# linum-uqam/ViT-OCM-WMSegmentation

Hardware: AMD Instinct MI355X
Metric: OCM tiles/s (224x224, ViT-S/16 attention-map inference) (higher is better)
Workload: dtype bf16x3

## Files before the change

### include/ocm_vit.h

```cpp
#ifndef OCM_VIT_H
#define OCM_VIT_H

#include <stddef.h>
#include <stdint.h>

#ifdef __cplusplus
extern "C" {
#endif

#define OCM_ABI_VERSION 20

enum {
    OCM_OK = 0,
    OCM_EINVAL = 1,
    OCM_ESTATE = 2,
    OCM_EHIP = 3,
    OCM_ENOMEM = 4,
    OCM_ENAME = 5
};

enum {
    OCM_PREC_BF16 = 0,
    OCM_PREC_FP32 = 1,
    OCM_PREC_BF16X3 = 2
// ... 101 lines not shown
int ocm_linear_resid_ln_supported(int32_t D);
int ocm_op_linear_resid_ln(int32_t precision, const void *a, const void *w, const float *bias, const float *resid,
                           float *x, const float *gamma, const float *beta, void *xn, int32_t M, int32_t D, int32_t K,
                           float eps, void *stream);

enum { OCM_GEMM_LINEAR = 0, OCM_GEMM_QKV = 1, OCM_GEMM_LINEAR_LD = 2, OCM_GEMM_CONV = 3, OCM_GEMM_RESID_LN = 4 };
enum { OCM_PLAN_STATS_EPILOGUE = 1, OCM_PLAN_SPLITK_OFFERED = 2, OCM_PLAN_CONV3X3 = 4 };
typedef struct ocm_gemm_plan_info {
    int32_t bm, bn;
    int32_t waves;
    int32_t mfma16;
    int32_t lds_dma;
    int32_t stages;
    int32_t ksteps;
    int32_t splitk;
} ocm_gemm_plan_info;
int ocm_gemm_plan(int32_t family, int32_t precision, int32_t epilogue, int32_t M, int32_t N, int32_t K, uint32_t flags,
                  ocm_gemm_plan_info *plan);

int32_t ocm_n_pad(int32_t n_tokens);
int32_t ocm_n_pad_prec(int32_t precision, int32_t n_tokens);

int ocm_op_qkv_proj(int32_t precision, const void *a, const void *w, const float *bias, void *q, void *k,
                    void *vt, float *qkv_f32, int32_t batch, int32_t n_tokens, int32_t heads,
                    void *stream);

int ocm_op_attention(int32_t precision, const void *q, const void *k, const void *vt, void *ctx, float *lse2,
                     int32_t batch, int32_t n_tokens, int32_t heads, float scale, void *stream);

int ocm_op_attention_probs(int32_t precision, const void *q, const void *k, const float *lse2, float *attn,
                           int32_t batch, int32_t n_tokens, int32_t heads, float scale,
                           void *stream);

int ocm_op_attention_rows(int32_t precision, const void *q, const void *k, const int32_t *query_rows,
                          int32_t n_rows, float *rows, int32_t batch, int32_t n_tokens, int32_t heads, float scale,
                          void *stream);

int ocm_op_qkv_proj_hd(int32_t precision, const void *a, const void *w, const float *bias, void *q, void *k, void *vt,
                       float *qkv_f32, int32_t batch, int32_t n_tokens, int32_t heads, int32_t head_dim, void *stream);
int ocm_op_attention_hd(int32_t precision, const void *q, const void *k, const void *vt, void *ctx, float *lse2,
                        int32_t batch, int32_t n_tokens, int32_t heads, int32_t head_dim, float scale, void *stream);
int ocm_op_attention_probs_hd(int32_t precision, const void *q, const void *k, const float *lse2, float *attn,
                              int32_t batch, int32_t n_tokens, int32_t heads, int32_t head_dim, float scale, void *stream);

enum {
    OCM_ATTN_BF16_WHOLE = 0,
    OCM_ATTN_BF16_STREAM = 1,
    OCM_ATTN_FP32_STREAM = 2,
    OCM_ATTN_X3_WAVE_SPLIT = 3,
    OCM_ATTN_X3_PIPELINED = 4,
    OCM_ATTN_X3_DMA = 5,
    OCM_ATTN_X3_DMA_KSPLIT = 6
};
typedef struct ocm_attention_plan_info {
    int32_t kernel;
    int32_t waves;
    int32_t stages;
    int32_t kslices;
    int32_t grid_x, grid_y, grid_z;
    int32_t lds_bytes;
    uint64_t workspace_need;
} ocm_attention_plan_info;
int ocm_attention_plan(int32_t precision, int32_t batch, int32_t n_tokens, int32_t heads, int32_t head_dim, size_t workspace_bytes,
                       ocm_attention_plan_info *plan);

size_t ocm_attention_workspace_bytes(int32_t precision, int32_t batch, int32_t n_tokens, int32_t heads, int32_t head_dim);
// ... 231 lines not shown
```

### vit-ocm-wmsegmentation_amd/_lib.py

```python
import ctypes as C
import os

_HERE = os.path.dirname(os.path.abspath(__file__))
LIB_PATH = os.environ.get("OCM_VIT_LIB") or os.path.join(_HERE, "libocm_vit.so")

OCM_ABI_VERSION = 20
OCM_OK, OCM_EINVAL, OCM_ESTATE, OCM_EHIP, OCM_ENOMEM, OCM_ENAME = 0, 1, 2, 3, 4, 5

OCM_PREC_BF16 = 0
OCM_PREC_FP32 = 1
OCM_PREC_BF16X3 = 2
OCM_SWIN_OPT_FUSE_MLP = 0
OCM_SWIN_CFG_BACKBONE = 1
OCM_SWIN_OUT_HIDDEN, OCM_SWIN_OUT_RESHAPED, OCM_SWIN_OUT_ATTENTION = 0, 1, 2
PRECISIONS = {"bf16": OCM_PREC_BF16, "fp32": OCM_PREC_FP32, "bf16x3": OCM_PREC_BF16X3}
DEFAULT_PRECISION = "bf16x3"
OCM_LN_F32, OCM_LN_BF16, OCM_LN_SPLIT = 0, 1, 2
OCM_OPT_FUSE_LN = 0
OCM_OPT_FOLD_LN = 1

OCM_OUT_FEAT = 1 << 0
OCM_OUT_ATTN = 1 << 1
OCM_OUT_QKV = 1 << 2
OCM_OUT_TOKENS = 1 << 3
# ... 109 lines not shown
    "ocm_abi_version": (C.c_int, []),
    "ocm_last_error": (C.c_char_p, []),
    "ocm_vit_create": (C.c_int, [C.POINTER(OcmVitConfig), C.POINTER(_vp)]),
    "ocm_vit_destroy": (None, [_vp]),
    "ocm_vit_set_param": (C.c_int, [_vp, C.c_char_p, _vp, _sz, _vp]),
    "ocm_vit_params_ready": (C.c_int, [_vp]),
    "ocm_vit_workspace_bytes": (_sz, [_vp, _i32, _i32]),
    "ocm_vit_forward": (C.c_int, [_vp, C.POINTER(OcmVitIO)]),
    "ocm_vit_prepare_tokens": (C.c_int, [_vp, C.POINTER(OcmVitIO), _vp]),
    "ocm_vit_block_forward": (C.c_int, [_vp, _i32, _vp, _i32, _i32, _i32, _vp, _vp, _vp, _sz, _vp]),
    "ocm_vit_final_norm": (C.c_int, [_vp, _vp, _vp, _i64, _vp]),
    "ocm_op_layernorm": (C.c_int, [_vp, _vp, _vp, _vp, _i32, _i64, _i32, _f32, _vp]),
    "ocm_op_cast_bf16": (C.c_int, [_vp, _vp, _sz, _vp]),
    "ocm_op_cast_split": (C.c_int, [_vp, _vp, _sz, _vp]),
    "ocm_op_merge_split": (C.c_int, [_vp, _vp, _sz, _vp]),
    "ocm_n_pad_prec": (_i32, [_i32, _i32]),
    "ocm_op_linear": (C.c_int, [_i32, _vp, _vp, _vp, _vp, _vp, _i32, _i32, _i32, _i32, _vp]),
    "ocm_op_linear_stats": (C.c_int, [_i32, _vp, _vp, _vp, _vp, _vp, _vp, _vp, _vp, _vp, _i32, _i32, _i32, _vp]),
    "ocm_linear_resid_ln_supported": (C.c_int, [_i32]),
    "ocm_op_linear_resid_ln": (C.c_int, [_i32, _vp, _vp, _vp, _vp, _vp, _vp, _vp, _vp, _i32, _i32, _i32, _f32, _vp]),
    "ocm_gemm_plan": (C.c_int, [_i32, _i32, _i32, _i32, _i32, _i32, C.c_uint32, C.POINTER(OcmGemmPlanInfo)]),
    "ocm_n_pad": (_i32, [_i32]),
    "ocm_op_qkv_proj": (C.c_int, [_i32, _vp, _vp, _vp, _vp, _vp, _vp, _vp, _i32, _i32, _i32, _vp]),
    "ocm_op_attention": (C.c_int, [_i32, _vp, _vp, _vp, _vp, _vp, _i32, _i32, _i32, _f32, _vp]),
    "ocm_op_qkv_proj_hd": (C.c_int, [_i32, _vp, _vp, _vp, _vp, _vp, _vp, _vp, _i32, _i32, _i32, _i32, _vp]),
    "ocm_op_attention_hd": (C.c_int, [_i32, _vp, _vp, _vp, _vp, _vp, _i32, _i32, _i32, _i32, _f32, _vp]),
    "ocm_op_attention_probs_hd": (C.c_int, [_i32, _vp, _vp, _vp, _vp, _i32, _i32, _i32, _i32, _f32, _vp]),
    "ocm_attention_plan": (C.c_int, [_i32, _i32, _i32, _i32, _i32, _sz, C.POINTER(OcmAttentionPlanInfo)]),
    "ocm_attention_workspace_bytes": (_sz, [_i32, _i32, _i32, _i32, _i32]),
    "ocm_op_attention_ws": (C.c_int, [_i32, _vp, _vp, _vp, _vp, _vp, _i32, _i32, _i32, _i32, _f32, _vp, _sz, _vp]),
    "ocm_op_attention_generic": (C.c_int, [C.c_int32, C.c_void_p, C.c_void_p, C.c_void_p, C.c_int32, C.c_int32, C.c_int32,
                                           C.c_int32, C.c_float, C.c_void_p]),
    "ocm_op_attention_probs": (C.c_int, [_i32, _vp, _vp, _vp, _vp, _i32, _i32, _i32, _f32, _vp]),
    "ocm_op_attention_rows": (C.c_int, [_i32, _vp, _vp, _vp, _i32, _vp, _i32, _i32, _i32, _f32, _vp]),
    "ocm_op_attention_map": (C.c_int, [_vp, _vp, _i32, _i32, _i32, _i32, _i32, _i32, _i32, _vp]),
    "ocm_op_tile_postprocess": (C.c_int, [_vp, _vp, _i32, _i32, _i32, _i32, _vp]),
    "ocm_op_bilinear_upsample": (C.c_int, [_vp, _vp, _i32, _i32, _i32, _i32, _vp]),
    "ocm_op_nearest_upsample": (C.c_int, [_vp, _vp, _i32, _i32, _i32, _i32, _vp]),
    "ocm_op_stitch": (C.c_int, [_vp, _vp, _vp, _i32, _i32, _i32, _vp]),
    "ocm_op_normalize_u8": (C.c_int, [_vp, _i64, _vp, _vp, _vp, _vp]),
    "ocm_otsu_threshold": (_i32, [C.POINTER(C.c_uint64), _i64]),
    "ocm_op_threshold_u8": (C.c_int, [_vp, _vp, _i64, _i32, _vp]),
    "ocm_vit_graph_stats": (C.c_int, [C.c_void_p, C.POINTER(C.c_uint64), C.POINTER(C.c_uint64)]),
    "ocm_swin_create": (C.c_int, [C.POINTER(OcmSwinConfig), C.POINTER(C.c_void_p)]),
    "ocm_swin_destroy": (None, [C.c_void_p]),
    "ocm_swin_set_param": (C.c_int, [C.c_void_p, C.c_char_p, C.c_void_p, C.c_size_t, C.c_void_p]),
    "ocm_swin_params_ready": (C.c_int, [C.c_void_p]),
    "ocm_swin_workspace_bytes": (C.c_size_t, [C.c_void_p, C.c_int32]),
    "ocm_swin_forward": (C.c_int, [C.c_void_p, C.c_void_p, C.c_int32, C.c_void_p, C.c_void_p, C.c_void_p, C.c_void_p,
                                   C.c_size_t, C.c_void_p]),
    "ocm_swin_forward_ex": (C.c_int, [C.c_void_p, C.c_void_p, C.c_int32, C.c_void_p, C.c_void_p, C.c_void_p,
                                      C.POINTER(OcmSwinOutputs), C.c_void_p, C.c_size_t, C.c_void_p]),
    "ocm_swin_output_shape": (C.c_int, [C.POINTER(OcmSwinConfig), C.c_int32, C.c_int32, C.c_int32, C.POINTER(C.c_int64)]),
    "ocm_swin_set_option": (C.c_int, [C.c_void_p, C.c_int32, C.c_int32]),
    "ocm_op_swin_window_probs": (C.c_int, [C.c_int32, C.c_void_p, C.c_int32, C.c_void_p, C.c_void_p, C.c_void_p, C.c_int32,
                                           C.c_int32, C.c_int32, C.c_int32, C.c_int32, C.c_int32, C.c_void_p]),
    "ocm_swin_window_scratch_floats": (C.c_size_t, [C.c_int32, C.c_int32]),
    "ocm_op_swin_tokens_to_nchw": (C.c_int, [C.c_void_p, C.c_void_p, C.c_int32, C.c_int32, C.c_int32, C.c_void_p]),
    "ocm_op_swin_lnqkv": (C.c_int, [C.c_int32, C.c_void_p, C.c_void_p, C.c_void_p, C.c_void_p, C.c_void_p, C.c_void_p,
                                    C.c_int64, C.c_int32, C.c_float, C.c_void_p]),
    "ocm_op_swin_mlp": (C.c_int, [C.c_int32, C.c_void_p, C.c_void_p, C.c_void_p, C.c_void_p, C.c_void_p, C.c_void_p,
                                  C.c_void_p, C.c_int64, C.c_int32, C.c_int32, C.c_float, C.c_void_p]),
    "ocm_op_swin_attn_block": (C.c_int, [C.c_int32, C.c_void_p, C.c_void_p, C.c_void_p, C.c_void_p, C.c_void_p, C.c_void_p,
                                         C.c_void_p, C.c_void_p, C.c_void_p, C.c_int32, C.c_int32, C.c_int32, C.c_int32,
                                         C.c_int32, C.c_int32, C.c_float, C.c_void_p]),
    "ocm_op_swin_window_attention": (C.c_int, [C.c_int32, C.c_void_p, C.c_int32, C.c_void_p, C.c_int32, C.c_void_p,
# ... 143 lines not shown
```

### vit-ocm-wmsegmentation_amd/csrc/attn_plan.h

```cpp
#pragma once
#include <cstddef>

enum AttnKernel : int {
    ATTN_BF16_WHOLE = 0,
    ATTN_BF16_STREAM = 1,
    ATTN_F32_STREAM = 2,
    ATTN_X3_WS = 3,
    ATTN_X3_PP = 4,
    ATTN_X3_DMA = 5,
    ATTN_X3_DMA_KSPLIT = 6,
};

struct AttnPlan {
    AttnKernel kernel;
    int waves;
    int stages;
    int kslices;
    unsigned grid_x, grid_y, grid_z;
    int lds_bytes;
    size_t workspace_need;
};

constexpr int ATTN_QTILE = 32;
constexpr int ATTN_BF16_WHOLE_MAX_N = 256;
constexpr int ATTN_X3_WIDE_MIN_N = 1024;
constexpr int ATTN_X3_WS_MAX_WGS = 128;
constexpr int ATTN_KSPLIT_MAX = 4, ATTN_KSPLIT_WGS_4 = 64, ATTN_KSPLIT_WGS_3 = 96, ATTN_KSPLIT_WGS_2 = 128;
constexpr int ATTN_KSPLIT_ROW_FLOATS = 64 + 4;
constexpr int ATTN_WS_LDS = 4 * 2 * 2 * 8192;
constexpr int ATTN_F32_LDS_PER_CHANNEL = 4 * 256;

constexpr int attn_qtiles(int n_tokens) { return (n_tokens + ATTN_QTILE - 1) / ATTN_QTILE; }
constexpr long attn_wide_wgs(int batch, int n_tokens, int heads) { return (long)((attn_qtiles(n_tokens) + 7) / 8) * batch * heads; }
constexpr size_t attn_ksplit_slice_bytes(int batch, int n_tokens, int heads) {
    return (size_t)batch * heads * n_tokens * ATTN_KSPLIT_ROW_FLOATS * sizeof(float);
}

constexpr size_t attn_plan_workspace_bytes(int prec, int batch, int n_tokens, int heads, int head_dim) {
    if (prec != 2 || head_dim != 64 || n_tokens <= ATTN_X3_WIDE_MIN_N) return 0;
    if (attn_wide_wgs(batch, n_tokens, heads) > ATTN_KSPLIT_WGS_2) return 0;
    return ATTN_KSPLIT_MAX * attn_ksplit_slice_bytes(batch, n_tokens, heads);
}

inline AttnPlan attn_plan(int prec, int batch, int n_tokens, int heads, int head_dim, size_t workspace_bytes) {
    const int qtiles = attn_qtiles(n_tokens);
    const unsigned bh = (unsigned)(batch * heads), gx4 = (unsigned)((qtiles + 3) / 4);
    if (prec == 0) {
        if (head_dim == 64 && n_tokens <= ATTN_BF16_WHOLE_MAX_N) return AttnPlan{ATTN_BF16_WHOLE, 8, 1, 1, bh, 1, 1, 0, 0};
        return AttnPlan{ATTN_BF16_STREAM, 4, 2, 1, gx4, bh, 1, 0, 0};
    }
    if (prec == 1) return AttnPlan{ATTN_F32_STREAM, 4, 2, 1, gx4, bh, 1, ATTN_F32_LDS_PER_CHANNEL * head_dim, 0};
    if (head_dim == 128) return AttnPlan{ATTN_X3_DMA, 4, 2, 1, gx4, bh, 1, 0, 0};
    if (n_tokens > ATTN_X3_WIDE_MIN_N) {
        const unsigned gx8 = (unsigned)((qtiles + 7) / 8);
        if (workspace_bytes) {
            const long wgs = (long)gx8 * bh;
            const int want = wgs <= ATTN_KSPLIT_WGS_4 ? 4 : wgs <= ATTN_KSPLIT_WGS_3 ? 3 : wgs <= ATTN_KSPLIT_WGS_2 ? 2 : 1;
            const int per = (qtiles + want - 1) / want, nslice = (qtiles + per - 1) / per;
            const size_t need = (size_t)nslice * attn_ksplit_slice_bytes(batch, n_tokens, heads);
            if (nslice > 1 && need <= workspace_bytes) return AttnPlan{ATTN_X3_DMA_KSPLIT, 8, 3, nslice, gx8, bh, (unsigned)nslice, 0, need};
        }
        return AttnPlan{ATTN_X3_DMA, 8, 3, 1, gx8, bh, 1, 0, 0};
    }
// ... 4 lines not shown
```

### vit-ocm-wmsegmentation_amd/csrc/engine.hip

```cpp
#include <stdarg.h>
#include <stdio.h>
#include <string.h>

#include <atomic>
#include <mutex>
#include <string>
#include <vector>

#include "host_common.h"
#include "launch.h"
#include "attn_plan.h"
#include "otsu.h"

static thread_local std::string g_err;

int ocm_fail(int code, const char *fmt, ...) {
    char buf[512];
    va_list ap;
    va_start(ap, fmt);
    vsnprintf(buf, sizeof buf, fmt, ap);
    va_end(ap);
    g_err = buf;
    return code;
}
// ... 322 lines not shown
    w.bytes = off;
    return w;
}

extern "C" size_t ocm_vit_workspace_bytes(const ocm_vit_t *h, int32_t batch, int32_t n_tokens) {
    if (!h || batch <= 0 || n_tokens <= 1) return 0;
    return carve(h, batch, n_tokens, nullptr).bytes;
}

static int check_ws(const ocm_vit *h, int batch, int n, void *ws, size_t ws_bytes) {
    if (!ws) return fail(OCM_ENOMEM, "workspace is null");
    if ((uintptr_t)ws & 255) return fail(OCM_EINVAL, "workspace must be 256-byte aligned");
    const size_t need = carve(h, batch, n, nullptr).bytes;
    if (ws_bytes < need) return fail(OCM_ENOMEM, "workspace too small: %zu < %zu bytes", ws_bytes, need);
    return OCM_OK;
}

static int run_attention(const ocm_vit *h, const Workspace &w, int batch, int n, bool attn_only, float *out_attn, float *out_qkv,
                         const int32_t *query_rows, int n_rows, float *out_rows, const char *qkv_w, const float *qkv_b,
                         const LnFold &ln, hipStream_t s) {
    const int H = h->H, np = ocm_n_pad_for(h->prec, n), pc = h->prec;
    const float scale = h->cfg.qk_scale;
    const bool want_v = !(attn_only && !out_qkv);
    if (!h->mfma_heads()) {
        float *qkv = out_qkv ? out_qkv : w.qkv32;
        { PROF(OCM_K_QKV, s); HIP_TRY(launch_qkv(pc, w.xn, qkv_w, qkv_b, nullptr, nullptr, nullptr, qkv, batch, n, np, H, h->hd, want_v, s, ln)); }
        { PROF(OCM_K_ATTN, s); HIP_TRY(launch_attention_generic(pc, qkv, attn_only ? nullptr : w.ctx, out_attn, query_rows, n_rows, out_rows, batch, n, H, h->hd, scale, s)); }
        return OCM_OK;
    }
    void *vt_dst = want_v ? w.vt : nullptr;
    { PROF(OCM_K_QKV, s); HIP_TRY(launch_qkv(pc, w.xn, qkv_w, qkv_b, w.q, w.k, vt_dst, out_qkv, batch, n, np, H, h->hd, want_v, s, ln)); }
    if (out_rows && !out_attn) { PROF(OCM_K_PROBS, s); HIP_TRY(launch_attention_rows(pc, w.q, w.k, query_rows, n_rows, out_rows, batch, n, np, H, scale, s, h->hd)); }
    if (attn_only && !out_attn) return OCM_OK;
    { PROF(OCM_K_ATTN, s); HIP_TRY(launch_attention(pc, w.q, w.k, w.vt, attn_only ? nullptr : w.ctx, out_attn ? w.lse : nullptr, batch, n, np, H, scale, s, h->hd, w.kpart, w.kpart_bytes)); }
    if (out_attn) {
        PROF(OCM_K_PROBS, s);
        HIP_TRY(launch_attention_probs(pc, w.q, w.k, w.lse, out_attn, batch, n, np, H, scale, s, h->hd, query_rows, n_rows, out_rows));
    }
    return OCM_OK;
}

static int run_block(const ocm_vit *h, int i, const Workspace &w, float *x, int batch, int n, bool attn_only,
                     float *out_attn, float *out_qkv, const int32_t *query_rows, int n_rows, float *out_rows,
                     hipStream_t s, bool xn_ready = false, const float *next_g = nullptr, const float *next_b = nullptr,
                     bool *xn_out = nullptr) {
    const BlockP &bp = h->blk[i];
    const int D = h->D, T = batch * n;
    const float eps = h->cfg.ln_eps;
    const int pc = h->prec, lnk = ln_kind_of_prec(pc);
    const long t128 = (long)((T + 127) / 128) * (D / 128);
    const int fuse_opt = h->opt[OCM_OPT_FUSE_LN];
    const bool fuse_ln = linear_resid_ln_supported(D) && fuse_opt != 1 && ((T >= 8192 && t128 < 512) || fuse_opt == 2);
    if (xn_out) *xn_out = false;
    if (!xn_ready) { PROF(OCM_K_LN, s); HIP_TRY(launch_layernorm(x, h->ptr<float>(bp.ln1_g), h->ptr<float>(bp.ln1_b), w.xn, lnk, T, D, eps, s)); }
    if (int rc = run_attention(h, w, batch, n, attn_only, out_attn, out_qkv, query_rows, n_rows, out_rows, h->ptr<char>(bp.qkv_w),
                               h->ptr<float>(bp.qkv_b), LnFold(), s))
        return rc;
    if (attn_only) return OCM_OK;
    if (fuse_ln) {
        PROF(OCM_K_PROJ, s);
        HIP_TRY(launch_linear_resid_ln(pc, w.ctx, h->ptr<char>(bp.proj_w), h->ptr<float>(bp.proj_b), x, x, h->ptr<float>(bp.ln2_g), h->ptr<float>(bp.ln2_b), w.xn, T, D, D, eps, s));
    } else {
        { PROF(OCM_K_PROJ, s); HIP_TRY(launch_linear(pc, w.ctx, h->ptr<char>(bp.proj_w), h->ptr<float>(bp.proj_b), x, x, T, D, D, OCM_EPI_BIAS_RESID_F32, s)); }
        { PROF(OCM_K_LN, s); HIP_TRY(launch_layernorm(x, h->ptr<float>(bp.ln2_g), h->ptr<float>(bp.ln2_b), w.xn, lnk, T, D, eps, s)); }
    }
    { PROF(OCM_K_FC1, s); HIP_TRY(launch_linear(pc, w.xn, h->ptr<char>(bp.fc1_w), h->ptr<float>(bp.fc1_b), nullptr, w.hid, T, h->M, D, OCM_EPI_BIAS_GELU_BF16, s)); }
    if (fuse_ln && next_g && next_b) {
        PROF(OCM_K_FC2, s);
        HIP_TRY(launch_linear_resid_ln(pc, w.hid, h->ptr<char>(bp.fc2_w), h->ptr<float>(bp.fc2_b), x, x, next_g, next_b, w.xn, T, D, h->M, eps, s));
        if (xn_out) *xn_out = true;
// ... 407 lines not shown

extern "C" int ocm_op_attention_ws(int32_t precision, const void *q, const void *k, const void *vt, void *ctx, float *lse2,
                                   int32_t batch, int32_t n_tokens, int32_t heads, int32_t head_dim, float scale,
                                   void *workspace, size_t workspace_bytes, void *stream) {
    return op_attention(precision, q, k, vt, ctx, lse2, batch, n_tokens, heads, head_dim, scale, stream, workspace, workspace_bytes);
}

extern "C" int ocm_op_attention_generic(int32_t precision, const float *qkv_f32, void *ctx, float *attn, int32_t batch,
                                        int32_t n_tokens, int32_t heads, int32_t head_dim, float scale, void *stream) {
    int pc = 0, rc = prec_of(precision, &pc);
    if (rc) return rc;
    if (!qkv_f32 || (!ctx && !attn)) return fail(OCM_EINVAL, "null argument");
    if (batch <= 0 || n_tokens <= 0 || heads <= 0 || head_dim <= 0) return fail(OCM_EINVAL, "bad shape");
    if (head_dim % 4 || head_dim > 512 || n_tokens > 8192 || (pc == 2 && (heads * head_dim) % 32))
        return fail(OCM_EINVAL, "generic attention: head_dim %d must be a multiple of 4 up to 512, at most 8192 tokens, and "
                                "heads * head_dim a multiple of 32 for a split-bf16 context", head_dim);
    if ((int64_t)batch * heads > 65535) return fail(OCM_EINVAL, "batch * heads = %lld > 65535", (long long)batch * heads);
    HIP_TRY(launch_attention_generic(pc, qkv_f32, ctx, attn, nullptr, 0, nullptr, batch, n_tokens, heads, head_dim, scale,
                                     (hipStream_t)stream));
    return OCM_OK;
}

extern "C" int ocm_op_attention_probs(int32_t precision, const void *q, const void *k, const float *lse2, float *attn,
                                      int32_t batch, int32_t n_tokens, int32_t heads, float scale, void *stream) {
    return op_attention_probs(precision, q, k, lse2, attn, batch, n_tokens, heads, 64, scale, stream);
}

extern "C" int ocm_op_attention_probs_hd(int32_t precision, const void *q, const void *k, const float *lse2, float *attn,
                                         int32_t batch, int32_t n_tokens, int32_t heads, int32_t head_dim, float scale,
                                         void *stream) {
    return op_attention_probs(precision, q, k, lse2, attn, batch, n_tokens, heads, head_dim, scale, stream);
}

extern "C" int ocm_op_attention_rows(int32_t precision, const void *q, const void *k, const int32_t *query_rows,
                                     int32_t n_rows, float *rows, int32_t batch, int32_t n_tokens, int32_t heads,
                                     float scale, void *stream) {
    int pc = 0, rc = prec_of(precision, &pc);
    if (rc) return rc;
    if (!q || !k || !rows) return fail(OCM_EINVAL, "null argument");
    if (batch <= 0 || n_tokens <= 1 || heads <= 0 || n_rows <= 0) return fail(OCM_EINVAL, "bad shape");
    HIP_TRY(launch_attention_rows(pc, q, k, query_rows, n_rows, rows, batch, n_tokens, ocm_n_pad_for(pc, n_tokens), heads, scale,
                                  (hipStream_t)stream));
    return OCM_OK;
}

extern "C" int ocm_op_attention_map(const float *attn, float *maps, int32_t b, int32_t heads, int32_t n_tokens,
                                    int32_t query, int32_t hf, int32_t wf, int32_t p, void *stream) {
    if (!attn || !maps) return fail(OCM_EINVAL, "null argument");
    if (hf * wf + 1 != n_tokens) return fail(OCM_EINVAL, "hf*wf+1 = %d != n_tokens %d", hf * wf + 1, n_tokens);
    if (query < 0 || query >= n_tokens) return fail(OCM_EINVAL, "query %d out of range", query);
    HIP_TRY(launch_attention_map(attn, maps, b, heads, n_tokens, query, hf, wf, p, (hipStream_t)stream));
    return OCM_OK;
}

extern "C" int ocm_op_tile_postprocess(const float *rows, float *maps, int32_t tiles, int32_t heads, int32_t n_rows,
                                       int32_t pixels, void *stream) {
    if (!rows || !maps) return fail(OCM_EINVAL, "null argument");
    if (tiles <= 0 || heads <= 0 || n_rows <= 0 || pixels <= 0) return fail(OCM_EINVAL, "bad shape");
    HIP_TRY(launch_tile_postprocess(rows, maps, tiles, heads, n_rows, pixels, (hipStream_t)stream));
    return OCM_OK;
}

extern "C" int ocm_op_bilinear_upsample(const float *src, float *dst, int32_t tiles, int32_t h, int32_t w,
                                        int32_t scale, void *stream) {
    if (!src || !dst) return fail(OCM_EINVAL, "null argument");
    if (tiles <= 0 || h <= 0 || w <= 0 || scale <= 0) return fail(OCM_EINVAL, "bad shape");
// ... 162 lines not shown
```

### vit-ocm-wmsegmentation_amd/csrc/kernels_attn.hip

```cpp
#include <stdlib.h>

#include "launch.h"

#define LOG2E 1.4426950408889634f
#include "attn_plan.h"
#define OCM_VMCNT_ATTN(n) asm volatile("s_waitcnt vmcnt(%0)" ::"n"(n) : "memory")

#ifndef OCM_DEFER_MAX
#define OCM_DEFER_MAX 8.0f
#endif
__device__ __forceinline__ float defer_max_update(float &m, float cand) {
    if (__any(cand > m + OCM_DEFER_MAX)) {
        const float mn = fmaxf(m, cand);
        const float alpha = fast_exp2(m - mn);
        m = mn;
        return alpha;
    }
    return 1.0f;
}

template <bool WANT_O, int HD = 64>
__global__ __launch_bounds__(256, HD == 64 ? 3 : 2) void attn_fwd_kernel(const bf16 *__restrict__ Q, const bf16 *__restrict__ Kk,
                                                       const bf16 *__restrict__ Vt, bf16 *__restrict__ ctx,
                                                       float *__restrict__ lse2, int N, int npad, int H,
// ... 1196 lines not shown
#pragma unroll
    for (int e = 0; e < 16; ++e) lr[e] = lse2[(int64_t)bh * N + min(q0 + acc_row32(e, h), N - 1)];
    float *out = attn + (int64_t)bh * N * N;
    const int nkt = (N + 31) >> 5, per = (nkt + (int)gridDim.z - 1) / (int)gridDim.z;
    const int kt0 = (int)blockIdx.z * per, ktiles = min(nkt, kt0 + per);
    if (kt0 >= ktiles) return;
    bf16x8 kh[NQ], kl[NQ], nh[NQ], nl[NQ];
    loadrow(Kb, min(kt0 * 32 + r, N - 1), kh, kl);
    for (int kt = kt0; kt < ktiles; ++kt) {
        if (kt + 1 < ktiles) loadrow(Kb, min((kt + 1) * 32 + r, N - 1), nh, nl);
        f32x16 S;
#pragma unroll
        for (int e = 0; e < 16; ++e) S[e] = 0.f;
#pragma unroll
        for (int s = 0; s < NQ; ++s) S = mfma32x3(qh[s], ql[s], kh[s], kl[s], S);
        const int key = kt * 32 + r;
        if (key < N) {
#pragma unroll
            for (int e = 0; e < 16; ++e) {
                const int qrow = q0 + acc_row32(e, h);
                if (qrow < N) out[(int64_t)qrow * N + key] = fast_exp2(S[e] * scale2 - lr[e]);
            }
        }
#pragma unroll
        for (int s = 0; s < NQ; ++s) {
            kh[s] = nh[s];
            kl[s] = nl[s];
        }
    }
}

constexpr int PROBS_FOLD_ROWS = 8;

__global__ __launch_bounds__(256) void attn_probs_x3_span_kernel(const char *__restrict__ Q, const char *__restrict__ Kk,
                                                                 const float *__restrict__ lse2, float *__restrict__ attn,
                                                                 int N, int npad, float scale2,
                                                                 const int32_t *__restrict__ query_rows, int n_rows,
                                                                 float *__restrict__ rows) {
    constexpr int HD = 64, NQ = HD / 16, ROWB = HD * 4, PITCH = ROWB + 16, REGION = 32 * PITCH, TILEB = 32 * ROWB;
    __shared__ __attribute__((aligned(16))) char smem[4 * REGION];
    const int tid = threadIdx.x, lane = tid & 63, wave = tid >> 6;
    const int r = lane & 31, h = lane >> 5;
    int qblk, bh;
    xcd_remap2(qblk, bh);
    const int q0 = qblk * 32, nq = min(32, N - q0);
    const int nkt = (N + 31) >> 5;
    const char *Qb = Q + ((int64_t)bh * npad + q0) * ROWB;
    const char *Kb = Kk + (int64_t)bh * npad * ROWB;
    f32x4 qraw[2], kraw[2][8];
#pragma unroll
    for (int i = 0; i < 2; ++i) qraw[i] = *(const f32x4 *)(Qb + (i * 256 + tid) * 16);
#pragma unroll
    for (int t = 0; t < 2; ++t)
        if (wave + 4 * t < nkt) {
#pragma unroll
            for (int i = 0; i < 8; ++i) kraw[t][i] = *(const f32x4 *)(Kb + (int64_t)(wave + 4 * t) * TILEB + (i * 64 + lane) * 16);
        }
    float lr[16];
#pragma unroll
    for (int e = 0; e < 16; ++e) lr[e] = lse2[(int64_t)bh * N + min(q0 + acc_row32(e, h), N - 1)];
    auto stage = [&](char *region, int piece, const f32x4 &v) {
        *(f32x4 *)(region + (piece >> 4) * PITCH + (piece & 15) * 16) = v;
    };
    auto fragments = [&](const char *region, bf16x8(&hi)[NQ], bf16x8(&lo)[NQ]) {
        const char *rp = region + r * PITCH;
#pragma unroll
        for (int s = 0; s < NQ; ++s) {
            const char *p = rp + (s >> 1) * 128 + ((s & 1) * 16 + 8 * h) * 2;
            hi[s] = *(const bf16x8 *)p;
            lo[s] = *(const bf16x8 *)(p + 64);
        }
    };
    bf16x8 qh[NQ], ql[NQ];
#pragma unroll
    for (int i = 0; i < 2; ++i) stage(smem, i * 256 + tid, qraw[i]);
    lds_barrier();
    fragments(smem, qh, ql);
    lds_barrier();
    char *mine = smem + wave * REGION;
    float pr[2][16];
#pragma unroll
    for (int t = 0; t < 2; ++t) {
        const bool have = wave + 4 * t < nkt;
        if (have) {
#pragma unroll
            for (int i = 0; i < 8; ++i) stage(mine, i * 64 + lane, kraw[t][i]);
        }
        lds_barrier();
        if (have) {
            bf16x8 kh[NQ], kl[NQ];
            fragments(mine, kh, kl);
            f32x16 S;
#pragma unroll
            for (int e = 0; e < 16; ++e) S[e] = 0.f;
#pragma unroll
            for (int s = 0; s < NQ; ++s) S = mfma32x3(qh[s], ql[s], kh[s], kl[s], S);
#pragma unroll
            for (int e = 0; e < 16; ++e) pr[t][e] = fast_exp2(S[e] * scale2 - lr[e]);
        }
        lds_barrier();
    }
    float *span = attn + ((int64_t)bh * N + q0) * N;
    const int shift = (int)(((uintptr_t)span >> 2) & 3);
    float *img = (float *)smem + shift;
#pragma unroll
    for (int t = 0; t < 2; ++t) {
        const int key = (wave + 4 * t) * 32 + r;
        if (key < N) {
#pragma unroll
            for (int e = 0; e < 16; ++e) {
                const int row = acc_row32(e, h);
                if (row < nq) img[row * N + key] = pr[t][e];
            }
        }
    }
    lds_barrier();
    const int len = nq * N;
    const int lead = min((4 - shift) & 3, len), nvec = (len - lead) >> 2, tail = lead + 4 * nvec;
    if (tid < lead) span[tid] = img[tid];
    for (int i = tid; i < nvec; i += 256) *(f32x4 *)(span + lead + 4 * i) = *(const f32x4 *)(img + lead + 4 * i);
    if (tid < len - tail) span[tail + tid] = img[tail + tid];
    if (rows) {
        for (int i = 0; i < n_rows; ++i) {
            const int query = query_rows ? query_rows[i] : 0;
            if (query < q0 || query >= q0 + nq) continue;
            float *dst = rows + ((int64_t)bh * n_rows + i) * (N - 1);
            const float *src = img + (query - q0) * N + 1;
            for (int j = tid; j < N - 1; j += 256) dst[j] = src[j];
        }
    }
}


__device__ __forceinline__ void store_ctx1(int prec, char *rowp, int col, float v) {
    if (prec == 0) {
        *(bf16 *)(rowp + col * 2) = (bf16)v;
    } else if (prec == 1) {
        *(float *)(rowp + col * 4) = v;
    } else {
        bf16 hi, lo;
        split1(v, hi, lo);
        *(bf16 *)(rowp + sp_off(col)) = hi;
        *(bf16 *)(rowp + sp_off(col) + 64) = lo;
    }
}
// ... 159 lines not shown
            attn_merge_x3_kernel<64><<<dim3((unsigned)((rows + 15) / 16)), dim3(256), 0, s>>>(
                ksplit_ws, p.kslices, (char *)ctx, lse2, batch * heads, n_tokens, heads);
            break;
        }
    }
    return hipGetLastError();
}

template <int HD>
static hipError_t launch_probs_hd(int prec, const void *q, const void *k, const float *lse2, float *attn, int n_tokens, int n_pad,
                                  float scale2, dim3 grid, dim3 gridz, hipStream_t s) {
    const dim3 block(256);
    if (prec == 2)
        attn_probs_x3_kernel<HD><<<gridz, block, 0, s>>>((const char *)q, (const char *)k, lse2, attn, n_tokens, n_pad, scale2);
    else if (prec)
        attn_probs_f32_kernel<HD><<<grid, block, 0, s>>>((const float *)q, (const float *)k, lse2, attn, n_tokens, n_pad, scale2);
    else
        attn_probs_kernel<HD><<<grid, block, 0, s>>>((const bf16 *)q, (const bf16 *)k, lse2, attn, n_tokens, n_pad, scale2);
    return hipGetLastError();
}

hipError_t launch_attention_probs(int prec, const void *q, const void *k, const float *lse2, float *attn, int batch,
                                  int n_tokens, int n_pad, int heads, float scale, hipStream_t s, int head_dim,
                                  const int32_t *query_rows, int n_rows, float *rows) {
    if (head_dim != 64 && head_dim != 128) return hipErrorInvalidValue;
    const int qtiles = (n_tokens + 31) / 32;
    const dim3 grid((qtiles + 3) / 4, batch * heads);
    const int wgs = (int)(grid.x * grid.y), ktiles = qtiles;
    const int nz = wgs >= 256 ? 1 : min(ktiles, min(16, (512 + wgs - 1) / wgs));
    const dim3 gridz(grid.x, grid.y, nz);
    if (n_rows <= 0) rows = nullptr;
    bool folded = false;
    hipError_t e;
    if (prec == 2 && head_dim == 64 && n_tokens <= 255 && n_pad % 32 == 0 && n_pad >= n_tokens) {
        folded = rows && n_rows <= PROBS_FOLD_ROWS;
        attn_probs_x3_span_kernel<<<dim3(qtiles, batch * heads), dim3(256), 0, s>>>(
            (const char *)q, (const char *)k, lse2, attn, n_tokens, n_pad, scale * LOG2E, query_rows, n_rows, folded ? rows : nullptr);
        e = hipGetLastError();
    } else if (head_dim == 128) {
        e = launch_probs_hd<128>(prec, q, k, lse2, attn, n_tokens, n_pad, scale * LOG2E, grid, gridz, s);
    } else {
        e = launch_probs_hd<64>(prec, q, k, lse2, attn, n_tokens, n_pad, scale * LOG2E, grid, gridz, s);
    }
    if (e != hipSuccess || !rows || folded) return e;
    return launch_rows_from_probs(attn, query_rows, n_rows, rows, batch, n_tokens, heads, s);
}

__device__ __forceinline__ void load8(const bf16 *rowp, int c, float (&o)[8]) {
    const bf16x8 t = *(const bf16x8 *)(rowp + c * 8);
#pragma unroll
    for (int e = 0; e < 8; ++e) o[e] = (float)t[e];
}
__device__ __forceinline__ void load8(const float *rowp, int c, float (&o)[8]) {
    const f32x4 a = *(const f32x4 *)(rowp + c * 8), b = *(const f32x4 *)(rowp + c * 8 + 4);
#pragma unroll
    for (int e = 0; e < 4; ++e) {
        o[e] = a[e];
        o[4 + e] = b[e];
    }
}
__device__ __forceinline__ void load8(const sp32 *rowp, int c, float (&o)[8]) {
    const char *p = (const char *)rowp + sp_off(c * 8);
    const bf16x8 hi = *(const bf16x8 *)p, lo = *(const bf16x8 *)(p + 64);
#pragma unroll
    for (int e = 0; e < 8; ++e) o[e] = (float)hi[e] + (float)lo[e];
}

template <class E, int HD>
__global__ __launch_bounds__(64) void attn_rows_kernel(const E *__restrict__ Q, const E *__restrict__ Kk,
                                                       const int32_t *__restrict__ query_rows, int n_rows,
                                                       float *__restrict__ rows, int N, int npad, float scale2) {
    extern __shared__ __attribute__((aligned(16))) char smem[];
    float *sc = (float *)smem;
    const int lane = threadIdx.x, bh = blockIdx.y, qi = blockIdx.x;
    const int query = query_rows ? query_rows[qi] : 0;
    const E *qp = Q + ((int64_t)bh * npad + query) * HD;
// ... 111 lines not shown
```

### vit-ocm-wmsegmentation_amd/csrc/launch.h

```cpp
#pragma once
#include <atomic>
#include "common.h"
#include "gemm_plan.h"

typedef std::atomic<unsigned long long> OptinMask;
static inline hipError_t lds_optin(const void *kern, int bytes, OptinMask &done) {
    int dev = 0;
    if (hipError_t e = hipGetDevice(&dev); e != hipSuccess) return e;
    const unsigned long long bit = 1ull << (dev & 63);
    if (done.load(std::memory_order_acquire) & bit) return hipSuccess;
    const hipError_t e = hipFuncSetAttribute(kern, hipFuncAttributeMaxDynamicSharedMemorySize, bytes);
    if (e == hipSuccess) done.fetch_or(bit, std::memory_order_release);
    return e;
}

constexpr int OCM_WT_MASK = 35;

hipError_t launch_layernorm(const float *x, const float *gamma, const float *beta, void *y, int out_kind,
                            int64_t rows, int dim, float eps, hipStream_t s);
static inline int ln_kind_of_prec(int prec) { return prec == 0 ? 1 : prec == 1 ? 0 : 2; }
hipError_t launch_cast_bf16(const float *src, bf16 *dst, size_t count, hipStream_t s);
hipError_t launch_cast_split(const float *src, void *dst, size_t count, hipStream_t s);
hipError_t launch_merge_split(const void *src, float *dst, size_t count, hipStream_t s);
hipError_t launch_fold_split(const float *src, void *dst, int D, int C, int pp, hipStream_t s);
// ... 27 lines not shown
                          float *dvec, int N, int K, hipStream_t s);

hipError_t launch_linear(int prec, const void *a, const void *w, const float *bias, const float *resid, void *out, int M,
                         int N, int K, int epilogue, hipStream_t s, const LnFold &ln = LnFold(),
                         const StatsOut &so = StatsOut());
bool linear_resid_ln_supported(int D);
hipError_t launch_linear_resid_ln(int prec, const void *a, const void *w, const float *bias, const float *resid, float *x,
                                  const float *gamma, const float *beta, void *xn, int M, int D, int K, float eps,
                                  hipStream_t s);
hipError_t launch_qkv(int prec, const void *a, const void *w, const float *bias, void *q, void *k, void *vt,
                      float *qkv_f32, int batch, int n_tokens, int n_pad, int heads, int head_dim, bool want_v,
                      hipStream_t s, const LnFold &ln = LnFold());
hipError_t launch_attention_generic(int prec, const float *qkv, void *ctx, float *attn, const int32_t *query_rows,
                                    int n_rows, float *rows, int batch, int n_tokens, int heads, int head_dim, float scale,
                                    hipStream_t s);
struct PatchArgs {
    const float *image;
    int64_t sb, sc, sy;
    const int32_t *origins;
    int batch, hp, wp, p, chans;
    const float *mask = nullptr;
    const float *mask_tok = nullptr;
};
hipError_t launch_patch_embed(int prec, const PatchArgs &pa, const void *w, const float *bias, const float *pos,
                              float *x, int dim, hipStream_t s, const StatsOut &so = StatsOut());

hipError_t launch_attention(int prec, const void *q, const void *k, const void *vt, void *ctx, float *lse2, int batch,
                            int n_tokens, int n_pad, int heads, float scale, hipStream_t s, int head_dim = 64,
                            float *ksplit_ws = nullptr, size_t ksplit_bytes = 0);
size_t attention_ksplit_bytes(int prec, int batch, int n_tokens, int heads, int head_dim);
hipError_t launch_attention_probs(int prec, const void *q, const void *k, const float *lse2, float *attn, int batch,
                                  int n_tokens, int n_pad, int heads, float scale, hipStream_t s, int head_dim = 64,
                                  const int32_t *query_rows = nullptr, int n_rows = 0, float *rows = nullptr);
hipError_t launch_rows_from_probs(const float *attn, const int32_t *query_rows, int n_rows, float *rows, int batch,
                                  int n_tokens, int heads, hipStream_t s);
hipError_t launch_attention_rows(int prec, const void *q, const void *k, const int32_t *query_rows, int n_rows,
                                 float *rows, int batch, int n_tokens, int n_pad, int heads, float scale, hipStream_t s,
                                 int head_dim = 64);
hipError_t launch_attention_map(const float *attn, float *maps, int b, int heads, int n_tokens, int query, int hf,
                                int wf, int p, hipStream_t s);

hipError_t launch_tile_postprocess(const float *rows, float *maps, int tiles, int heads, int n_rows, int pixels,
                                   hipStream_t s);
hipError_t launch_bilinear_up(const float *src, float *dst, int tiles, int h, int w, int scale, hipStream_t s);
hipError_t launch_nearest_up(const float *src, float *dst, int tiles, int h, int w, int rep, hipStream_t s);
hipError_t launch_stitch(const float *crops, float *out, const double *ramp, int n, int window, int stride,
                         hipStream_t s);
hipError_t launch_normalize_u8(const float *img, size_t count, float *part, uint8_t *out,
                               unsigned long long *hist256, hipStream_t s);
hipError_t launch_threshold_u8(const uint8_t *img, uint8_t *mask, size_t count, int thresh, hipStream_t s);
hipError_t launch_tokens_to_fmap(const float *y, float *out, int batch, int n_tokens, int dim, hipStream_t s);
hipError_t launch_pixel_shuffle(const float *lin, float *out, int batch, int hp, int wp, int c_out, int sh, hipStream_t s);
hipError_t launch_head_mean(const float *rows, float *maps, int tiles, int heads, int n_rows, int pixels, hipStream_t s);
hipError_t launch_image_to_gray_u8(const float *img, int64_t stride_c, int chans, size_t count, uint8_t *out,
                                   unsigned long long *hist256, hipStream_t s);
hipError_t launch_blend_u8(const uint8_t *img, const uint8_t *att, size_t count, double alpha, double one_minus_alpha,
                           uint8_t *out, unsigned long long *hist256, hipStream_t s);

hipError_t launch_stitch_image_u8(const float *image, int64_t sc, int64_t sy, int chans, int H, int W, uint8_t *out,
                                  const double *ramp, int n, int window, int stride, unsigned long long *hist256,
                                  hipStream_t s);
hipError_t launch_weighted_u8(const float *heat, const uint8_t *img, size_t count, float *part, uint8_t *result,
                              uint8_t *att_u8, unsigned long long *hist_res, unsigned long long *hist_att, hipStream_t s);
hipError_t launch_histogram_u8(const uint8_t *img, size_t count, unsigned long long *hist256, hipStream_t s);
hipError_t launch_median_filter(const float *src, float *dst, int tiles, int h, int w, int k, hipStream_t s);
hipError_t launch_downscale_centre(const float *src, float *dst, int tiles, int h, int w, int f, hipStream_t s);
// ... 42 lines not shown
```

Before: 30030.

## Compute attention maps in one pass with in-kernel softmax statistics

Adds a template variant of the split-bf16 span probability kernel that computes each row's max and sum itself instead of reading a log-sum-exp buffer from the preceding flash-attention pass. It swaps the MFMA operand order so each row's keys sit across lanes, reduces max and sum across waves through LDS, and writes normalized probabilities. When only attention maps are requested for short sequences (ViT-S/16 at 224 has 197 tokens), the separate attention kernel launch is skipped, removing a whole kernel and its K/V reads. The cost is extra LDS barriers and reductions inside the probs kernel, plus a different store pattern for the image.

Measured after the change: 30210 (median of 6 runs). No clear change (+0.6%).

```diff
diff --git a/include/ocm_vit.h b/include/ocm_vit.h
--- a/include/ocm_vit.h
+++ b/include/ocm_vit.h
@@ -157,6 +157,10 @@
                            int32_t batch, int32_t n_tokens, int32_t heads, float scale,
                            void *stream);
 
+int ocm_op_attention_maps(int32_t precision, const void *q, const void *k, float *attn, int32_t batch, int32_t n_tokens,
+                          int32_t heads, int32_t head_dim, float scale, const int32_t *query_rows, int32_t n_rows,
+                          float *rows, void *stream);
+
 int ocm_op_attention_rows(int32_t precision, const void *q, const void *k, const int32_t *query_rows,
                           int32_t n_rows, float *rows, int32_t batch, int32_t n_tokens, int32_t heads, float scale,
                           void *stream);
diff --git a/vit-ocm-wmsegmentation_amd/_lib.py b/vit-ocm-wmsegmentation_amd/_lib.py
--- a/vit-ocm-wmsegmentation_amd/_lib.py
+++ b/vit-ocm-wmsegmentation_amd/_lib.py
@@ -165,6 +165,7 @@
     "ocm_op_attention_generic": (C.c_int, [C.c_int32, C.c_void_p, C.c_void_p, C.c_void_p, C.c_int32, C.c_int32, C.c_int32,
                                            C.c_int32, C.c_float, C.c_void_p]),
     "ocm_op_attention_probs": (C.c_int, [_i32, _vp, _vp, _vp, _vp, _i32, _i32, _i32, _f32, _vp]),
+    "ocm_op_attention_maps": (C.c_int, [_i32, _vp, _vp, _vp, _i32, _i32, _i32, _i32, _f32, _vp, _i32, _vp, _vp]),
     "ocm_op_attention_rows": (C.c_int, [_i32, _vp, _vp, _vp, _i32, _vp, _i32, _i32, _i32, _f32, _vp]),
     "ocm_op_attention_map": (C.c_int, [_vp, _vp, _i32, _i32, _i32, _i32, _i32, _i32, _i32, _vp]),
     "ocm_op_tile_postprocess": (C.c_int, [_vp, _vp, _i32, _i32, _i32, _i32, _vp]),
diff --git a/vit-ocm-wmsegmentation_amd/csrc/attn_plan.h b/vit-ocm-wmsegmentation_amd/csrc/attn_plan.h
--- a/vit-ocm-wmsegmentation_amd/csrc/attn_plan.h
+++ b/vit-ocm-wmsegmentation_amd/csrc/attn_plan.h
@@ -29,6 +29,11 @@
 constexpr int ATTN_KSPLIT_ROW_FLOATS = 64 + 4;
 constexpr int ATTN_WS_LDS = 4 * 2 * 2 * 8192;
 constexpr int ATTN_F32_LDS_PER_CHANNEL = 4 * 256;
+
+constexpr int ATTN_MAPS_SPAN_MAX_N = 255;
+constexpr bool attn_maps_one_pass(int prec, int head_dim, int n_tokens) {
+    return prec == 2 && head_dim == 64 && n_tokens >= 1 && n_tokens <= ATTN_MAPS_SPAN_MAX_N;
+}
 
 constexpr int attn_qtiles(int n_tokens) { return (n_tokens + ATTN_QTILE - 1) / ATTN_QTILE; }
 constexpr long attn_wide_wgs(int batch, int n_tokens, int heads) { return (long)((attn_qtiles(n_tokens) + 7) / 8) * batch * heads; }
diff --git a/vit-ocm-wmsegmentation_amd/csrc/engine.hip b/vit-ocm-wmsegmentation_amd/csrc/engine.hip
--- a/vit-ocm-wmsegmentation_amd/csrc/engine.hip
+++ b/vit-ocm-wmsegmentation_amd/csrc/engine.hip
@@ -378,10 +378,17 @@
     { PROF(OCM_K_QKV, s); HIP_TRY(launch_qkv(pc, w.xn, qkv_w, qkv_b, w.q, w.k, vt_dst, out_qkv, batch, n, np, H, h->hd, want_v, s, ln)); }
     if (out_rows && !out_attn) { PROF(OCM_K_PROBS, s); HIP_TRY(launch_attention_rows(pc, w.q, w.k, query_rows, n_rows, out_rows, batch, n, np, H, scale, s, h->hd)); }
     if (attn_only && !out_attn) return OCM_OK;
-    { PROF(OCM_K_ATTN, s); HIP_TRY(launch_attention(pc, w.q, w.k, w.vt, attn_only ? nullptr : w.ctx, out_attn ? w.lse : nullptr, batch, n, np, H, scale, s, h->hd, w.kpart, w.kpart_bytes)); }
+    const bool one_pass = out_attn && attn_maps_one_pass(pc, h->hd, n);
+    if (!(attn_only && one_pass)) {
+        PROF(OCM_K_ATTN, s);
+        HIP_TRY(launch_attention(pc, w.q, w.k, w.vt, attn_only ? nullptr : w.ctx, out_attn && !one_pass ? w.lse : nullptr, batch, n, np, H, scale, s, h->hd, w.kpart, w.kpart_bytes));
+    }
     if (out_attn) {
         PROF(OCM_K_PROBS, s);
-        HIP_TRY(launch_attention_probs(pc, w.q, w.k, w.lse, out_attn, batch, n, np, H, scale, s, h->hd, query_rows, n_rows, out_rows));
+        if (one_pass)
+            HIP_TRY(launch_attention_maps(pc, w.q, w.k, out_attn, batch, n, np, H, scale, s, h->hd, query_rows, n_rows, out_rows));
+        else
+            HIP_TRY(launch_attention_probs(pc, w.q, w.k, w.lse, out_attn, batch, n, np, H, scale, s, h->hd, query_rows, n_rows, out_rows));
     }
     return OCM_OK;
 }
@@ -855,6 +862,23 @@
     return op_attention_probs(precision, q, k, lse2, attn, batch, n_tokens, heads, head_dim, scale, stream);
 }
 
+extern "C" int ocm_op_attention_maps(int32_t precision, const void *q, const void *k, float *attn, int32_t batch,
+                                     int32_t n_tokens, int32_t heads, int32_t head_dim, float scale,
+                                     const int32_t *query_rows, int32_t n_rows, float *rows, void *stream) {
+    int pc = 0, rc = prec_of(precision, &pc);
+    if (rc) return rc;
+    if (!q || !k || !attn) return fail(OCM_EINVAL, "null argument");
+    if (batch <= 0 || n_tokens <= 0 || heads <= 0 || (int64_t)batch * heads > 65535) return fail(OCM_EINVAL, "bad shape");
+    if (!attn_maps_one_pass(pc, head_dim, n_tokens))
+        return fail(OCM_EINVAL, "one-pass attention maps are built for split-bf16 operands, 64-wide heads and at most %d tokens "
+                                "(precision %d, head_dim %d, n_tokens %d): use ocm_op_attention and ocm_op_attention_probs",
+                    ATTN_MAPS_SPAN_MAX_N, precision, head_dim, n_tokens);
+    if (rows && (n_rows <= 0 || n_tokens < 2)) return fail(OCM_EINVAL, "selected rows need n_rows >= 1 and n_tokens >= 2");
+    HIP_TRY(launch_attention_maps(pc, q, k, attn, batch, n_tokens, ocm_n_pad_for(pc, n_tokens), heads, scale, (hipStream_t)stream,
+                                  head_dim, query_rows, rows ? n_rows : 0, rows));
+    return OCM_OK;
+}
+
 extern "C" int ocm_op_attention_rows(int32_t precision, const void *q, const void *k, const int32_t *query_rows,
                                      int32_t n_rows, float *rows, int32_t batch, int32_t n_tokens, int32_t heads,
                                      float scale, void *stream) {
diff --git a/vit-ocm-wmsegmentation_amd/csrc/kernels_attn.hip b/vit-ocm-wmsegmentation_amd/csrc/kernels_attn.hip
--- a/vit-ocm-wmsegmentation_amd/csrc/kernels_attn.hip
+++ b/vit-ocm-wmsegmentation_amd/csrc/kernels_attn.hip
@@ -1252,6 +1252,7 @@
 
 constexpr int PROBS_FOLD_ROWS = 8;
 
+template <bool OWN_STATS>
 __global__ __launch_bounds__(256) void attn_probs_x3_span_kernel(const char *__restrict__ Q, const char *__restrict__ Kk,
                                                                  const float *__restrict__ lse2, float *__restrict__ attn,
                                                                  int N, int npad, float scale2,
@@ -1277,8 +1278,10 @@
             for (int i = 0; i < 8; ++i) kraw[t][i] = *(const f32x4 *)(Kb + (int64_t)(wave + 4 * t) * TILEB + (i * 64 + lane) * 16);
         }
     float lr[16];
-#pragma unroll
-    for (int e = 0; e < 16; ++e) lr[e] = lse2[(int64_t)bh * N + min(q0 + acc_row32(e, h), N - 1)];
+    if constexpr (!OWN_STATS) {
+#pragma unroll
+        for (int e = 0; e < 16; ++e) lr[e] = lse2[(int64_t)bh * N + min(q0 + acc_row32(e, h), N - 1)];
+    }
     auto stage = [&](char *region, int piece, const f32x4 &v) {
         *(f32x4 *)(region + (piece >> 4) * PITCH + (piece & 15) * 16) = v;
     };
@@ -1314,23 +1317,71 @@
 #pragma unroll
             for (int e = 0; e < 16; ++e) S[e] = 0.f;
 #pragma unroll
-            for (int s = 0; s < NQ; ++s) S = mfma32x3(qh[s], ql[s], kh[s], kl[s], S);
-#pragma unroll
-            for (int e = 0; e < 16; ++e) pr[t][e] = fast_exp2(S[e] * scale2 - lr[e]);
+            for (int s = 0; s < NQ; ++s) {
+                if constexpr (OWN_STATS)
+                    S = mfma32x3(kh[s], kl[s], qh[s], ql[s], S);
+                else
+                    S = mfma32x3(qh[s], ql[s], kh[s], kl[s], S);
+            }
+#pragma unroll
+            for (int e = 0; e < 16; ++e) {
+                if constexpr (OWN_STATS)
+                    pr[t][e] = (wave + 4 * t) * 32 + acc_row32(e, h) < N ? S[e] * scale2 : -INFINITY;
+                else
+                    pr[t][e] = fast_exp2(S[e] * scale2 - lr[e]);
+            }
+        } else if constexpr (OWN_STATS) {
+#pragma unroll
+            for (int e = 0; e < 16; ++e) pr[t][e] = -INFINITY;
         }
         lds_barrier();
     }
     float *span = attn + ((int64_t)bh * N + q0) * N;
     const int shift = (int)(((uintptr_t)span >> 2) & 3);
     float *img = (float *)smem + shift;
-#pragma unroll
-    for (int t = 0; t < 2; ++t) {
-        const int key = (wave + 4 * t) * 32 + r;
-        if (key < N) {
+    if constexpr (OWN_STATS) {
+        float *stat = (float *)smem + 32 * 256;
+        float m = -INFINITY;
+#pragma unroll
+        for (int t = 0; t < 2; ++t)
+#pragma unroll
+            for (int e = 0; e < 16; ++e) m = fmaxf(m, pr[t][e]);
+        m = fmaxf(m, __shfl_xor(m, 32, 64));
+        if (h == 0) stat[wave * 32 + r] = m;
+        lds_barrier();
+        m = fmaxf(fmaxf(stat[r], stat[32 + r]), fmaxf(stat[64 + r], stat[96 + r]));
+        float l = 0.f;
+#pragma unroll
+        for (int t = 0; t < 2; ++t)
 #pragma unroll
             for (int e = 0; e < 16; ++e) {
-                const int row = acc_row32(e, h);
-                if (row < nq) img[row * N + key] = pr[t][e];
+                pr[t][e] = fast_exp2(pr[t][e] - m);
+                l += pr[t][e];
+            }
+        l += __shfl_xor(l, 32, 64);
+        if (h == 0) stat[128 + wave * 32 + r] = l;
+        lds_barrier();
+        l = ((stat[128 + r] + stat[160 + r]) + stat[192 + r]) + stat[224 + r];
+        const float inv = 1.0f / l;
+        if (r < nq) {
+#pragma unroll
+            for (int t = 0; t < 2; ++t)
+#pragma unroll
+                for (int e = 0; e < 16; ++e) {
+                    const int key = (wave + 4 * t) * 32 + acc_row32(e, h);
+                    if (key < N) img[r * N + key] = pr[t][e] * inv;
+                }
+        }
+    } else {
+#pragma unroll
+        for (int t = 0; t < 2; ++t) {
+            const int key = (wave + 4 * t) * 32 + r;
+            if (key < N) {
+#pragma unroll
+                for (int e = 0; e < 16; ++e) {
+                    const int row = acc_row32(e, h);
+                    if (row < nq) img[row * N + key] = pr[t][e];
+                }
             }
         }
     }
@@ -1556,9 +1607,9 @@
     if (n_rows <= 0) rows = nullptr;
     bool folded = false;
     hipError_t e;
-    if (prec == 2 && head_dim == 64 && n_tokens <= 255 && n_pad % 32 == 0 && n_pad >= n_tokens) {
+    if (attn_maps_one_pass(prec, head_dim, n_tokens) && n_pad % 32 == 0 && n_pad >= n_tokens) {
         folded = rows && n_rows <= PROBS_FOLD_ROWS;
-        attn_probs_x3_span_kernel<<<dim3(qtiles, batch * heads), dim3(256), 0, s>>>(
+        attn_probs_x3_span_kernel<false><<<dim3(qtiles, batch * heads), dim3(256), 0, s>>>(
             (const char *)q, (const char *)k, lse2, attn, n_tokens, n_pad, scale * LOG2E, query_rows, n_rows, folded ? rows : nullptr);
         e = hipGetLastError();
     } else if (head_dim == 128) {
@@ -1566,6 +1617,20 @@
     } else {
         e = launch_probs_hd<64>(prec, q, k, lse2, attn, n_tokens, n_pad, scale * LOG2E, grid, gridz, s);
     }
+    if (e != hipSuccess || !rows || folded) return e;
+    return launch_rows_from_probs(attn, query_rows, n_rows, rows, batch, n_tokens, heads, s);
+}
+
+hipError_t launch_attention_maps(int prec, const void *q, const void *k, float *attn, int batch, int n_tokens, int n_pad,
+                                 int heads, float scale, hipStream_t s, int head_dim, const int32_t *query_rows, int n_rows,
+                                 float *rows) {
+    if (!attn_maps_one_pass(prec, head_dim, n_tokens) || n_pad % 32 || n_pad < n_tokens) return hipErrorInvalidValue;
+    if ((int64_t)batch * heads > 65535) return hipErrorInvalidValue;
+    if (n_rows <= 0) rows = nullptr;
+    const bool folded = rows && n_rows <= PROBS_FOLD_ROWS;
+    attn_probs_x3_span_kernel<true><<<dim3((n_tokens + 31) / 32, batch * heads), dim3(256), 0, s>>>(
+        (const char *)q, (const char *)k, nullptr, attn, n_tokens, n_pad, scale * LOG2E, query_rows, n_rows, folded ? rows : nullptr);
+    const hipError_t e = hipGetLastError();
     if (e != hipSuccess || !rows || folded) return e;
     return launch_rows_from_probs(attn, query_rows, n_rows, rows, batch, n_tokens, heads, s);
 }
diff --git a/vit-ocm-wmsegmentation_amd/csrc/launch.h b/vit-ocm-wmsegmentation_amd/csrc/launch.h
--- a/vit-ocm-wmsegmentation_amd/csrc/launch.h
+++ b/vit-ocm-wmsegmentation_amd/csrc/launch.h
@@ -83,6 +83,9 @@
 hipError_t launch_attention_probs(int prec, const void *q, const void *k, const float *lse2, float *attn, int batch,
                                   int n_tokens, int n_pad, int heads, float scale, hipStream_t s, int head_dim = 64,
                                   const int32_t *query_rows = nullptr, int n_rows = 0, float *rows = nullptr);
+hipError_t launch_attention_maps(int prec, const void *q, const void *k, float *attn, int batch, int n_tokens, int n_pad,
+                                 int heads, float scale, hipStream_t s, int head_dim = 64,
+                                 const int32_t *query_rows = nullptr, int n_rows = 0, float *rows = nullptr);
 hipError_t launch_rows_from_probs(const float *attn, const int32_t *query_rows, int n_rows, float *rows, int batch,
                                   int n_tokens, int heads, hipStream_t s);
 hipError_t launch_attention_rows(int prec, const void *q, const void *k, const int32_t *query_rows, int n_rows,
```
